# tomerlieber/doc-agents

Measured on AMD Instinct MI355X. Metric: QA queries/sec + p50 cache-miss latency; docs/min ingest at 1/2/4/8 MI355X, higher is better.
Workload: dtype bf16

## Files before the change

docagents_amd/ops/csrc/decode_attn.hip:

```cpp
#include "common.h"
#include "decode_merge.h"

#include <cstdlib>
#include <type_traits>

#pragma clang fp contract(on)

constexpr int DEC_NT = 1;
constexpr int DEC_VEARLY = 2;
constexpr int DEC_PFT = 4;
constexpr int DEC_XC = 8;

struct DecRope {
  bf16_t* kc;
  bf16_t* vc;
  const float* cs;
  const int* pos;
};

template <int D, int G, int VAR>
__global__ void __launch_bounds__(256)
decode_attn_kernel(const bf16_t* __restrict__ q, int ldq, const bf16_t* __restrict__ kc,
                   const bf16_t* __restrict__ vc, const int* __restrict__ lens, const int* __restrict__ slot,
                   const int* __restrict__ pre,
// ... 407 lines not shown
#pragma unroll
      for (int ds = 0; ds < NDS; ++ds) sacc[t] = mfma16(__builtin_bit_cast(bf16x8_t, kr[t][ds]), qf[ds], sacc[t]);
    }
    float mx = -INFINITY;
#pragma unroll
    for (int t = 0; t < 4; ++t)
#pragma unroll
      for (int i = 0; i < 4; ++i) {
        const int key = 16 * t + 4 * fg + i;
        const float sc = key < nk ? sacc[t][i] * scale_log2e : -INFINITY;
        sacc[t][i] = sc;
        mx = fmaxf(mx, sc);
      }
    mx = fmaxf(mx, __shfl_xor(mx, 16, 64));
    mx = max_xhalf(mx);
    const float m_new = fmaxf(m_run, mx);
    const float m_use = (m_new == -INFINITY) ? 0.f : m_new;
    const float alpha = exp2f(m_run - m_use);
    m_run = m_new;
    float psum = 0.f;
#pragma unroll
    for (int t = 0; t < 4; ++t)
#pragma unroll
      for (int i = 0; i < 4; ++i) {
        const float p = __builtin_amdgcn_exp2f(sacc[t][i] - m_use);
        sacc[t][i] = p;
        psum += p;
      }
    l_part = l_part * alpha + psum;
#pragma unroll
    for (int i = 0; i < NDT; ++i) oacc[i] *= alpha;
    asm volatile("s_waitcnt vmcnt(0)" ::: "memory");
#pragma unroll
    for (int c = 0; c < 2; ++c) {
      const u32x4_t pw = u32x4_t{pack_bf2(sacc[2 * c][0], sacc[2 * c][1]), pack_bf2(sacc[2 * c][2], sacc[2 * c][3]),
                                 pack_bf2(sacc[2 * c + 1][0], sacc[2 * c + 1][1]),
                                 pack_bf2(sacc[2 * c + 1][2], sacc[2 * c + 1][3])};
      const bf16x8_t pb = __builtin_bit_cast(bf16x8_t, pw);
      const int q4 = fr >> 2, p4 = fr & 3;
#pragma unroll
      for (int dt = 0; dt < NDT; ++dt) {
        const int col = dt * 16 + 4 * p4;
        const int r0 = 32 * c + 4 * fg + q4, r1 = r0 + 16;
        const s16x4_t lo = lds_read_tr16(myv + r0 * (D * 2) + (((col >> 3) ^ vswz<D>(r0)) << 4) + (col & 7) * 2);
        const s16x4_t hi = lds_read_tr16(myv + r1 * (D * 2) + (((col >> 3) ^ vswz<D>(r1)) << 4) + (col & 7) * 2);
        const bf16x8_t va = bf16x8_t{lo[0], lo[1], lo[2], lo[3], hi[0], hi[1], hi[2], hi[3]};
        oacc[dt] = mfma16(va, pb, oacc[dt]);
      }
    }
    asm volatile("s_waitcnt lgkmcnt(0)" ::: "memory");
  }
  float l_tot = l_part + __shfl_xor(l_part, 16, 64);
  l_tot = sum_xhalf(l_tot);
  if (fg == 0) { swm[w][fr] = m_run; swl[w][fr] = l_tot; }
  __syncthreads();
  float* so = (float*)sv;
#pragma unroll
  for (int dt = 0; dt < NDT; ++dt)
#pragma unroll
    for (int i = 0; i < 4; ++i) so[(w * 16 + fr) * D + dt * 16 + 4 * fg + i] = oacc[dt][i];
  __syncthreads();
  for (int i = tid; i < G * D; i += 256) {
    const int g = i / D, d = i % D;
    const float M = fmaxf(fmaxf(swm[0][g], swm[1][g]), fmaxf(swm[2][g], swm[3][g]));
    const float Mu = (M == -INFINITY) ? 0.f : M;
    float o = 0.f, ls = 0.f;
#pragma unroll
    for (int ww = 0; ww < 4; ++ww) {
      const float f = exp2f(swm[ww][g] - Mu);
      o += so[(ww * 16 + g) * D + d] * f;
      ls += swl[ww][g] * f;
    }
    dec_store(o, M, ls, b, hk * G + g, d, H, nsplit, split, D, po, pm, pl, out, ldo);
  }
  __shared__ int s_last;
  dec_finish<D, G>(po, pm, pl, H, Hkv, nsplit, b, hk, cnt, out, ldo, &s_last);
}

template <int D>
__device__ __forceinline__ int vswz1(int r) {
  return D == 96 ? ((r >> 1) & 3) : vswz<D>(r);
}

template <int D, bool XC, bool RP>
__global__ void __launch_bounds__(256)
decode_attn_mfma1_kernel(const bf16_t* __restrict__ q, int ldq, const bf16_t* __restrict__ kc,
                         const bf16_t* __restrict__ vc, const int* __restrict__ lens, const int* __restrict__ slot,
                         const int* __restrict__ pre, int H, int Hkv, int max_seq, int chunk_max, int nsplit,
                         float scale_log2e, float* __restrict__ po, float* __restrict__ pm, float* __restrict__ pl,
                         bf16_t* __restrict__ out, int ldo, int* __restrict__ cnt, DecRope rope) {
  static_assert(D == 64 || D == 96 || D == 128, "head dim");
  constexpr int KT = 64, NDS = D / 32, NDT = D / 16, NS = D / 8;
  constexpr int VBYTES = KT * D * 2, NDMA = VBYTES / 1024;
  typedef __attribute__((address_space(3))) void* lds_ptr_t;
  typedef __attribute__((address_space(1))) const void* gptr_t;
  __shared__ __attribute__((aligned(16))) char sv[4 * 2 * VBYTES];
  __shared__ float swm[4], swl[4];

  int split = blockIdx.x, hk = blockIdx.y, b = blockIdx.z;
  if constexpr (XC) {
    const int wl = blockIdx.x + gridDim.x * (blockIdx.y + gridDim.y * blockIdx.z);
    const int s8 = wl >> 3, pair = (s8 / nsplit) * 8 + (wl & 7);
    split = s8 % nsplit;
    hk = pair % Hkv;
    b = pair / Hkv;
  }
  const int L = lens[b];
  DA_ASSERT(L >= 0 && L <= max_seq && slot[b] >= 0);
  const int chunk = dec_chunk(L, nsplit, chunk_max);
  DA_ASSERT(chunk <= 8 * KT);
  const int kstart = split * chunk;
  const bool own_new = RP && kstart <= L - 1 && L - 1 < kstart + chunk;
  const int kend = min(RP ? L - 1 : L, kstart + chunk);
  const int tid = threadIdx.x, lane = tid & 63, w = tid >> 6;
  const int fr = lane & 15, fg = lane >> 4;
  const size_t cbase = ((size_t)slot[b] * Hkv + hk) * (size_t)max_seq * D;
  const int P = pre ? pre[2 * b] : 0;
  const size_t pbase = P ? ((size_t)pre[2 * b + 1] * Hkv + hk) * (size_t)max_seq * D : cbase;
  DA_ASSERT(P >= 0 && P <= L);
  DA_ASSERT(!RP || rope.pos[b] == L - 1);

  const int ta = kstart + w * KT, tb = ta + 4 * KT;
  u32x4_t kr[2][4][NDS];
  auto issue_tile = [&](auto STR, int j, int t0) {
    constexpr bool S = decltype(STR)::value;
    const int nk = kend - t0;
    const bool shared = t0 < P;
    const bf16_t* kb = nk > 0 ? kc + (shared ? pbase : cbase) + (size_t)t0 * D : kc + cbase;
    const bf16_t* vb = nk > 0 ? vc + (shared ? pbase : cbase) + (size_t)t0 * D : vc + cbase;
    const int last = nk > 0 ? min(KT, nk) - 1 : 0;
    [[maybe_unused]] const int npre = P - t0;
    [[maybe_unused]] const bf16_t* ko = kc + cbase + (size_t)t0 * D;
    [[maybe_unused]] const bf16_t* vo = vc + cbase + (size_t)t0 * D;
#pragma unroll
    for (int t = 0; t < 4; ++t)
#pragma unroll
      for (int ds = 0; ds < NDS; ++ds) {
        const int key = min(16 * t + fr, last);
        const bf16_t* base = (S && key >= npre) ? ko : kb;
        kr[j][t][ds] = __builtin_nontemporal_load((const u32x4_t*)(base + (size_t)key * D + ds * 32 + fg * 8));
      }
    char* myv = sv + (w * 2 + j) * VBYTES;
#pragma unroll
    for (int i = 0; i < NDMA; ++i) {
      const int pc = i * 64 + lane, row = pc / NS, sl = pc % NS;
      const int c = sl ^ vswz1<D>(row);
      const int key = min(row, last);
      const bf16_t* base = (S && key >= npre) ? vo : vb;
      __builtin_amdgcn_global_load_lds((gptr_t)(base + (size_t)key * D + c * 8), (lds_ptr_t)(myv + i * 1024), 16, 0, 2);
    }
  };
  auto issue = [&](int j, int t0) {
    if (t0 < P && P < t0 + KT && t0 < kend) issue_tile(std::true_type{}, j, t0);
    else issue_tile(std::false_type{}, j, t0);
  };
  issue(0, ta);
  issue(1, tb);

  bf16x8_t qf[NDS];
  [[maybe_unused]] __shared__ __attribute__((aligned(16))) bf16_t sqb[RP ? D : 1];
  [[maybe_unused]] __shared__ float skn[RP ? D : 1], svn[RP ? D : 1];
  [[maybe_unused]] __shared__ float ssn;
  if constexpr (RP) {
    constexpr int HALF = D / 2;
    const bf16_t* qrow = q + (size_t)b * ldq;
    if (tid < D) {
      const int d = tid, i = d >> 1;
      const float c = rope.cs[((size_t)(L - 1) * HALF + i) * 2], sn = rope.cs[((size_t)(L - 1) * HALF + i) * 2 + 1];
      auto rot = [&](const bf16_t* hp) {
        const float x1 = bf2f(hp[d & ~1]), x2 = bf2f(hp[d | 1]);
        return f2bf((d & 1) ? x2 * c + x1 * sn : x1 * c - x2 * sn);
      };
      sqb[d] = rot(qrow + hk * D);
      if (own_new) {
        const bf16_t kn = rot(qrow + (size_t)(H + hk) * D), vn = qrow[(size_t)(H + Hkv + hk) * D + d];
        skn[d] = bf2f(kn);
        svn[d] = bf2f(vn);
        const size_t crow = cbase + (size_t)(L - 1) * D;
        rope.kc[crow + d] = kn;
        rope.vc[crow + d] = vn;
      }
    }
    __syncthreads();
#pragma unroll
    for (int ds = 0; ds < NDS; ++ds)
      qf[ds] = fr == 0 ? *(const bf16x8_t*)(sqb + ds * 32 + fg * 8) : bf16x8_t{0, 0, 0, 0, 0, 0, 0, 0};
    if (own_new && w == 0) {
      float part = 0.f;
      for (int d = lane; d < D; d += 64) part += bf2f(sqb[d]) * skn[d];
      part = wave_sum(part);
      if (lane == 0) ssn = part * scale_log2e;
    }
  } else {
#pragma unroll
    for (int ds = 0; ds < NDS; ++ds)
      qf[ds] = fr == 0 ? *(const bf16x8_t*)(q + (size_t)b * ldq + hk * D + ds * 32 + fg * 8)
                       : bf16x8_t{0, 0, 0, 0, 0, 0, 0, 0};
  }
  f32x4_t oacc[NDT];
#pragma unroll
  for (int i = 0; i < NDT; ++i) oacc[i] = f32x4_t{0.f, 0.f, 0.f, 0.f};
  float m_run = -INFINITY, l_part = 0.f;
  asm volatile("s_waitcnt vmcnt(0)" ::: "memory");

  auto process = [&](int j, int t0) {
    const int nk = kend - t0;
    f32x4_t sacc[4];
#pragma unroll
    for (int t = 0; t < 4; ++t) {
      sacc[t] = f32x4_t{0.f, 0.f, 0.f, 0.f};
#pragma unroll
      for (int ds = 0; ds < NDS; ++ds) sacc[t] = mfma16(__builtin_bit_cast(bf16x8_t, kr[j][t][ds]), qf[ds], sacc[t]);
    }
    float mx = -INFINITY;
#pragma unroll
    for (int t = 0; t < 4; ++t)
#pragma unroll
      for (int i = 0; i < 4; ++i) {
        const int key = 16 * t + 4 * fg + i;
        const float sc = key < nk ? sacc[t][i] * scale_log2e : -INFINITY;
        sacc[t][i] = sc;
        mx = fmaxf(mx, sc);
      }
    mx = fmaxf(mx, __shfl_xor(mx, 16, 64));
    mx = max_xhalf(mx);
    const float m_new = fmaxf(m_run, mx);
    const float m_use = (m_new == -INFINITY) ? 0.f : m_new;
    const float alpha = exp2f(m_run - m_use);
    m_run = m_new;
    float psum = 0.f;
#pragma unroll
    for (int t = 0; t < 4; ++t)
#pragma unroll
      for (int i = 0; i < 4; ++i) {
        const float p = __builtin_amdgcn_exp2f(sacc[t][i] - m_use);
        sacc[t][i] = p;
        psum += p;
      }
    l_part = l_part * alpha + psum;
#pragma unroll
    for (int i = 0; i < NDT; ++i) oacc[i] *= alpha;
    const char* myv = sv + (w * 2 + j) * VBYTES;
#pragma unroll
    for (int c = 0; c < 2; ++c) {
      const u32x4_t pw = u32x4_t{pack_bf2(sacc[2 * c][0], sacc[2 * c][1]), pack_bf2(sacc[2 * c][2], sacc[2 * c][3]),
                                 pack_bf2(sacc[2 * c + 1][0], sacc[2 * c + 1][1]),
                                 pack_bf2(sacc[2 * c + 1][2], sacc[2 * c + 1][3])};
      const bf16x8_t pb = __builtin_bit_cast(bf16x8_t, pw);
      const int q4 = fr >> 2, p4 = fr & 3;
#pragma unroll
      for (int dt = 0; dt < NDT; ++dt) {
        const int col = dt * 16 + 4 * p4;
        const int r0 = 32 * c + 4 * fg + q4, r1 = r0 + 16;
        const s16x4_t lo = lds_read_tr16(myv + r0 * (D * 2) + (((col >> 3) ^ vswz1<D>(r0)) << 4) + (col & 7) * 2);
        const s16x4_t hi = lds_read_tr16(myv + r1 * (D * 2) + (((col >> 3) ^ vswz1<D>(r1)) << 4) + (col & 7) * 2);
        const bf16x8_t va = bf16x8_t{lo[0], lo[1], lo[2], lo[3], hi[0], hi[1], hi[2], hi[3]};
        oacc[dt] = mfma16(va, pb, oacc[dt]);
      }
    }
  };
  if (ta < kend) process(0, ta);
  if (tb < kend) process(1, tb);

  float l_tot = l_part + __shfl_xor(l_part, 16, 64);
  l_tot = sum_xhalf(l_tot);
  if (lane == 0) { swm[w] = m_run; swl[w] = l_tot; }
  asm volatile("s_waitcnt lgkmcnt(0)" ::: "memory");
  __syncthreads();
  float* so = (float*)sv;
  if (fr == 0) {
#pragma unroll
    for (int dt = 0; dt < NDT; ++dt)
#pragma unroll
      for (int i = 0; i < 4; ++i) so[w * D + dt * 16 + 4 * fg + i] = oacc[dt][i];
  }
  __syncthreads();
  for (int d = tid; d < D; d += 256) {
    float M = fmaxf(fmaxf(swm[0], swm[1]), fmaxf(swm[2], swm[3]));
    if (own_new) M = fmaxf(M, ssn);
    const float Mu = (M == -INFINITY) ? 0.f : M;
    float o = 0.f, ls = 0.f;
#pragma unroll
    for (int ww = 0; ww < 4; ++ww) {
      const float f = exp2f(swm[ww] - Mu);
      o += so[ww * D + d] * f;
      ls += swl[ww] * f;
    }
    if (own_new) {
      const float f = exp2f(ssn - Mu);
      o += svn[d] * f;
      ls += f;
    }
    dec_store(o, M, ls, b, hk, d, H, nsplit, split, D, po, pm, pl, out, ldo);
  }
  __shared__ int s_last;
  dec_finish<D, 1, XC>(po, pm, pl, H, Hkv, nsplit, b, hk, cnt, out, ldo, &s_last);
}

constexpr int kDecPrefetchPairs = 32;
enum DecRoute { DEC_INVALID, DEC_MFMA1, DEC_MHA_STREAM, DEC_MHA_PREFETCH, DEC_MHA_PREFETCH_XC, DEC_GQA_MFMA, DEC_GQA_VALU };

static DecRoute dec_route(int D, int G, int pairs, int chunk, int nsplit, bool has_rope, bool xc, bool has_cnt,
                          bool mfma1_enabled) {
  const bool few = pairs <= kDecPrefetchPairs;
  if (G == 1) {
    if (xc && (!few || pairs % 8 || !has_cnt || nsplit < 2)) return DEC_INVALID;
    if (mfma1_enabled && few && chunk <= 512) return DEC_MFMA1;
    if (xc) return DEC_MHA_PREFETCH_XC;
    return few ? DEC_MHA_PREFETCH : DEC_MHA_STREAM;
  }
  if (xc || has_rope || (G != 2 && G != 4 && G != 8)) return DEC_INVALID;
  return D == 96 ? DEC_GQA_VALU : DEC_GQA_MFMA;
}

struct DecBf16Args : DecArgs {
  const bf16_t* kc; const bf16_t* vc;
  DecRope rope;
};

template <int D>
static int launch_decode(const DecBf16Args& a, DecRoute route, bool xc) {
#define VALU(GG, VAR) decode_attn_kernel<D, GG, VAR><<<a.grid, 256, 0, a.s>>>(a.q, a.ldq, a.kc, a.vc, DEC_KARGS(a), a.rope)
#define GQA(GG) decode_attn_gqa_kernel<D, GG><<<a.grid, 256, 0, a.s>>>(a.q, a.ldq, a.kc, a.vc, DEC_KARGS(a))
#define M1(XCV, RPV) decode_attn_mfma1_kernel<D, XCV, RPV><<<a.grid, 256, 0, a.s>>>(a.q, a.ldq, a.kc, a.vc, DEC_KARGS(a), a.rope)
  const bool rp = a.rope.cs != nullptr;
  switch (route) {
    case DEC_MFMA1:
      if (xc) { if (rp) M1(true, true); else M1(true, false); }
      else { if (rp) M1(false, true); else M1(false, false); }
      break;
    case DEC_MHA_STREAM: VALU(1, DEC_NT | DEC_VEARLY); break;
    case DEC_MHA_PREFETCH: VALU(1, DEC_NT | DEC_VEARLY | DEC_PFT); break;
    case DEC_MHA_PREFETCH_XC: VALU(1, DEC_NT | DEC_VEARLY | DEC_PFT | DEC_XC); break;
    case DEC_GQA_MFMA:
      if constexpr (D != 96) { if (a.G == 2) GQA(2); else if (a.G == 4) GQA(4); else GQA(8); }
      else return (int)hipErrorInvalidValue;
      break;
    case DEC_GQA_VALU:
      if constexpr (D == 96) { if (a.G == 2) VALU(2, DEC_NT); else if (a.G == 4) VALU(4, DEC_NT); else VALU(8, DEC_NT); }
      else return (int)hipErrorInvalidValue;
      break;
    default: return (int)hipErrorInvalidValue;
  }
#undef VALU
#undef GQA
#undef M1
  return (int)hipGetLastError();
}

DA_EXPORT int da_malloc_uncached(long long bytes, void** out) {
  hipError_t e = hipExtMallocWithFlags(out, (size_t)bytes, hipDeviceMallocUncached);
  if (e != hipSuccess) return (int)e;
  e = hipMemset(*out, 0, (size_t)bytes);
  if (e != hipSuccess) return (int)e;
  return (int)hipDeviceSynchronize();
}

DA_EXPORT int da_decode_attn(const void* q, int ldq, const void* k_cache, const void* v_cache, const void* lens,
                             const void* slot, const void* pre, int B, int H, int Hkv, int D, int max_seq, int chunk,
                             int nsplit, float scale, void* ws, void* o, int ldo, void* counters, const void* cos_sin,
                             const void* pos, int xc, void* stream) {
  DecBf16Args a;
  if (dec_fill(a, q, ldq, lens, slot, pre, B, H, Hkv, D, max_seq, chunk, nsplit, scale, ws, o, ldo, counters, cos_sin,
               pos, stream) || !k_cache || !v_cache)
    return (int)hipErrorInvalidValue;
  if (B == 0) return 0;
  a.kc = (const bf16_t*)k_cache; a.vc = (const bf16_t*)v_cache;
  a.rope = DecRope{(bf16_t*)k_cache, (bf16_t*)v_cache, (const float*)cos_sin, (const int*)pos};
  static const char* const m1 = getenv("DA_DECODE_MFMA1");
  const DecRoute route = dec_route(D, a.G, B * Hkv, chunk, nsplit, cos_sin != nullptr, xc != 0, counters != nullptr,
                                   !(m1 && m1[0] == '0'));
  const int err = D == 64 ? launch_decode<64>(a, route, xc != 0)
                  : D == 96 ? launch_decode<96>(a, route, xc != 0) : launch_decode<128>(a, route, xc != 0);
  return err ? err : dec_combine(a);
}
```

docagents_amd/ops/csrc/decode_merge.h:

```cpp
#pragma once
#include "common.h"

__device__ __forceinline__ int dec_chunk(int L, int nsplit, int chunk_arg) {
  const int c = ((L + nsplit - 1) / nsplit + 63) & ~63;
  return c < chunk_arg ? c : chunk_arg;
}

__device__ __forceinline__ void dec_store(float o, float M, float ls, int b, int h, int d, int H, int nsplit,
                                          int split, int D, float* po, float* pm, float* pl, bf16_t* out,
                                          int ldo) {
  if (nsplit == 1) {
    out[(size_t)b * ldo + h * D + d] = f2bf(ls > 0.f ? o / ls : 0.f);
    return;
  }
  const size_t pidx = ((size_t)b * H + h) * nsplit + split;
  po[pidx * D + d] = o;
  if (d == 0) { pm[pidx] = M; pl[pidx] = ls; }
}

template <int D, int G, bool XC = false>
__device__ __forceinline__ void dec_finish(const float* po, const float* pm, const float* pl, int H, int Hkv,
                                           int nsplit, int b, int hk, int* cnt, bf16_t* out, int ldo, int* s_last) {
  if (nsplit == 1 || cnt == nullptr) return;
  const int tid = threadIdx.x;
  asm volatile("s_waitcnt vmcnt(0)" ::: "memory");
  __syncthreads();
  if (tid == 0) {
    int* c = &cnt[b * Hkv + hk];
    const int old = XC ? __hip_atomic_fetch_add(c, 1, __ATOMIC_RELAXED, __HIP_MEMORY_SCOPE_AGENT) : atomicAdd(c, 1);
    *s_last = old == nsplit - 1;
    if (*s_last) {
      if constexpr (XC) __hip_atomic_store(c, 0, __ATOMIC_RELAXED, __HIP_MEMORY_SCOPE_AGENT);
      else *c = 0;
    }
  }
  __syncthreads();
  if (!*s_last) return;
  auto ld = [](const float* p) -> float {
    if constexpr (XC) return __hip_atomic_load(p, __ATOMIC_RELAXED, __HIP_MEMORY_SCOPE_AGENT);
    else return *p;
  };
  for (int i = tid; i < G * D; i += blockDim.x) {
    const int g = i / D, d = i % D, h = hk * G + g;
    const size_t base = ((size_t)b * H + h) * nsplit;
    float M = -INFINITY, lsum = 0.f, acc = 0.f;
    for (int s0 = 0; s0 < nsplit; s0 += 8) {
      float ms[8], ls[8], os[8];
#pragma unroll
      for (int j = 0; j < 8; ++j) {
        const int s = min(s0 + j, nsplit - 1);
        ms[j] = ld(pm + base + s);
        ls[j] = ld(pl + base + s);
        os[j] = ld(po + (base + s) * D + d);
      }
      float mx = M;
#pragma unroll
      for (int j = 0; j < 8; ++j)
        if (s0 + j < nsplit) mx = fmaxf(mx, ms[j]);
      const float mu = (mx == -INFINITY) ? 0.f : mx;
      const float r = (M == -INFINITY) ? 0.f : exp2f(M - mu);
      lsum *= r;
      acc *= r;
#pragma unroll
      for (int j = 0; j < 8; ++j) {
        if (s0 + j >= nsplit) continue;
        const float f = exp2f(ms[j] - mu);
        lsum += ls[j] * f;
        acc += os[j] * f;
      }
      M = mx;
    }
    out[(size_t)b * ldo + h * D + d] = f2bf(lsum > 0.f ? acc / lsum : 0.f);
  }
}

template <int D>
__global__ void decode_combine_kernel(const float* __restrict__ po, const float* __restrict__ pm,
                                      const float* __restrict__ pl, int H, int nsplit, bf16_t* __restrict__ o,
                                      int ldo) {
  const int b = blockIdx.y, h = blockIdx.x;
  const size_t base = ((size_t)b * H + h) * nsplit;
  float M = -INFINITY;
  for (int s = 0; s < nsplit; ++s) M = fmaxf(M, pm[base + s]);
  const float Mu = (M == -INFINITY) ? 0.f : M;
  float lsum = 0.f;
  for (int s = 0; s < nsplit; ++s) lsum += pl[base + s] * exp2f(pm[base + s] - Mu);
  const float inv = lsum > 0.f ? 1.f / lsum : 0.f;
  for (int d = threadIdx.x; d < D; d += blockDim.x) {
    float acc = 0.f;
    for (int s = 0; s < nsplit; ++s) acc += po[(base + s) * D + d] * exp2f(pm[base + s] - Mu);
    o[(size_t)b * ldo + h * D + d] = f2bf(acc * inv);
  }
}

struct DecArgs {
  const bf16_t* q; const int* lens; const int* slot; const int* pre;
  int ldq, B, H, Hkv, G, D, max_seq, chunk, nsplit, ldo;
  float sl2e;
  float* po; float* pm; float* pl;
  bf16_t* out; int* cnt;
  dim3 grid;
  hipStream_t s;
};
#define DEC_KARGS(a) (a).lens, (a).slot, (a).pre, (a).H, (a).Hkv, (a).max_seq, (a).chunk, (a).nsplit, (a).sl2e, (a).po, \
                     (a).pm, (a).pl, (a).out, (a).ldo, (a).cnt

static inline int dec_fill(DecArgs& a, const void* q, int ldq, const void* lens, const void* slot, const void* pre,
                           int B, int H, int Hkv, int D, int max_seq, int chunk, int nsplit, float scale, void* ws,
                           void* o, int ldo, void* counters, const void* cos_sin, const void* pos, void* stream) {
  bool ok = Hkv >= 1 && H % Hkv == 0 && chunk >= 64 && chunk % 64 == 0 && nsplit >= 1 && (D == 64 || D == 96 || D == 128);
  ok = ok && q && lens && slot && o && (nsplit == 1 || ws);
  ok = ok && (cos_sin == nullptr) == (pos == nullptr) && (!cos_sin || (H == Hkv && ldq >= (H + 2 * Hkv) * D));
  if (!ok) return (int)hipErrorInvalidValue;
  a.q = (const bf16_t*)q; a.lens = (const int*)lens; a.slot = (const int*)slot; a.pre = (const int*)pre;
  a.ldq = ldq; a.B = B; a.H = H; a.Hkv = Hkv; a.G = H / Hkv; a.D = D; a.max_seq = max_seq; a.chunk = chunk;
  a.nsplit = nsplit; a.ldo = ldo;
  a.sl2e = scale * 1.4426950408889634f;
  a.po = (float*)ws; a.pm = a.po + (size_t)B * H * nsplit * D; a.pl = a.pm + (size_t)B * H * nsplit;
  a.out = (bf16_t*)o; a.cnt = (int*)counters;
  a.grid = dim3(nsplit, Hkv, B); a.s = (hipStream_t)stream;
  return 0;
}

static inline int dec_combine(const DecArgs& a) {
  if (a.nsplit == 1 || a.cnt) return 0;
#define DEC_COMBINE(DD, NT) decode_combine_kernel<DD><<<dim3(a.H, a.B), NT, 0, a.s>>>(a.po, a.pm, a.pl, a.H, a.nsplit, a.out, a.ldo)
  if (a.D == 64) DEC_COMBINE(64, 64); else if (a.D == 96) DEC_COMBINE(96, 128); else DEC_COMBINE(128, 128);
#undef DEC_COMBINE
  DA_LAUNCH_CHECK();
}
```

docagents_amd/ops/kernels.py:

```python
from __future__ import annotations

import contextlib
import ctypes
import math
import os
import threading
from pathlib import Path

import torch

from . import gemm_plan
from .gemm_plan import (DK_MAX_M, DK_SPLITK_ABOVE, dk_fusable, dk_parts, dk_w8_fusable,
                        gemv_fusable, gemv_w4_fusable, gemv_w8_fusable, keeps_w4_copy, keeps_w8_copy,
                        prefill_w8_fusable, tile_w8_fusable, weight_op)
from .reference import (dequant_mxfp4, quant_weight_fp8, quant_weight_fp8_pow2,
                        quant_weight_mxfp4)

_LIB = None
_LOCK = threading.Lock()
_DEBUG = os.environ.get("DA_KERNELS_DEBUG", "0") == "1"
_LIB_PATH = Path(__file__).resolve().parent / ("_da_kernels_debug.so" if _DEBUG else "_da_kernels.so")

EPI_NONE, EPI_BIAS, EPI_GELU, EPI_SWIGLU, EPI_RESID = 0, 1, 2, 3, 4
EPI_ROPE = 6
# ... 773 lines not shown
    max_seq = 0
    if k_cache is not None:
        _i32(slot, "slot")
        _req(k_cache.is_contiguous() and v_cache.is_contiguous() and k_cache.shape == v_cache.shape, "caches")
        _req(k_cache.dim() == 4 and k_cache.shape[1] == Hkv and k_cache.shape[3] == D, "cache [S, Hkv, max_seq, D]")
        max_seq = k_cache.shape[2]
    _check(lib().da_rope_cache(_ptr(qkv), _ptr(pos), _ptr(slot), _ptr(cos_sin), _ptr(k_cache), _ptr(v_cache),
                               T, H, Hkv, D, max_seq, 1 if rotate_q else 0, _stream()), "rope_cache")
    return qkv


def flash_kv_cache_ok(D: int, causal: bool) -> bool:
    return causal and D == 96


def flash_attn_varlen(q, k, v, cu_seqlens, max_seqlen: int, H: int, Hkv: int, D: int, causal: bool,
                      scale: float | None = None, out=None, prefix=None, kv_cache=None, tail_only: bool = False):
    kc = vc = ks = kpos = None
    if kv_cache is not None:
        kc, vc, ks, kpos = kv_cache
        _req(flash_kv_cache_ok(D, causal), "kv_cache: causal D = 96 only")
        _bf16_cuda(kc, "k_cache"); _bf16_cuda(vc, "v_cache"); _i32(ks, "slot"); _i32(kpos, "pos")
        _req(kc.is_contiguous() and vc.is_contiguous() and kc.shape == vc.shape and kc.dim() == 4
             and kc.shape[1] == Hkv and kc.shape[3] == D, "caches [slots, Hkv, max_seq, D]")
        _req(ks.numel() >= q.shape[0] and kpos.numel() >= q.shape[0], "slot / pos per token")
        k = v = q
    for t, n in ((q, "q"), (k, "k"), (v, "v")):
        _bf16_cuda(t, n)
        _req(t.dim() == 2 and t.stride(1) == 1 and t.stride(0) % 8 == 0 and t.data_ptr() % 16 == 0, f"{n} layout")
    _i32(cu_seqlens, "cu_seqlens")
    _req(D in (32, 64, 96, 128), f"head dim {D} unsupported")
    _req(H % Hkv == 0, "H % Hkv")
    T = q.shape[0]
    if out is None:
        out = torch.empty((T, H * D), dtype=torch.bfloat16, device=q.device)
    scale = scale if scale is not None else 1.0 / math.sqrt(D)
    B = cu_seqlens.numel() - 1
    kp = vp = None
    hstride, P = 0, 0
    if prefix is not None:
        kp, vp, P = prefix
        P = int(P)
        _bf16_cuda(kp, "k_pre"); _bf16_cuda(vp, "v_pre")
        _req(kp.dim() == 3 and kp.shape == vp.shape and kp.shape[0] == Hkv and kp.shape[2] == D
             and kp.is_contiguous() and vp.is_contiguous() and 0 <= P <= kp.shape[1], "prefix K/V [Hkv, max_seq, D]")
        hstride = kp.shape[1] * D
    if kc is not None:
        _req(prefix is None or kp.shape[1] == kc.shape[2], "prefix and caches differ in max_seq")
        hstride = kc.shape[2] * D
    _check(lib().da_flash_attn_v2(_ptr(q), _ptr(k), _ptr(v), q.stride(0), k.stride(0), v.stride(0),
                                  _ptr(cu_seqlens), B, int(max_seqlen), H, Hkv, D, int(causal), float(scale),
                                  _ptr(out), out.stride(0), _ptr(kp), _ptr(vp), hstride, P, _ptr(ks), _ptr(kpos),
                                  _ptr(kc), _ptr(vc), int(bool(tail_only)), _stream()),
           "flash_attn_varlen")
    return out


_FUSED_COMBINE = True
_UC: dict = {}


class _RawBuf:

    def __init__(self, ptr: int, nbytes: int):
        self.ptr, self.nbytes = ptr, nbytes

    def data_ptr(self) -> int:
        return self.ptr


def _uncached(tag: str, nbytes: int, device) -> _RawBuf:
    key = (tag, device.index if device.index is not None else torch.cuda.current_device(),
           getattr(_ROLE, "name", "main"))
    bufs = _UC.setdefault(key, [])
    if not bufs or bufs[-1].nbytes < nbytes:
        n = max(nbytes, 1 << 20)
        p = ctypes.c_void_p()
        with torch.cuda.device(device):
            _check(lib().da_malloc_uncached(n, ctypes.byref(p)), "hipExtMallocWithFlags(uncached)")
        bufs.append(_RawBuf(p.value, n))
    return bufs[-1]


def _decode_split(B: int, Hkv: int, max_len: int, chunk: int):
    if chunk <= 0:
        want = max_len * B * Hkv / 768
        chunk = 512
        while chunk < want and chunk < 4096:
            chunk *= 2
    return chunk, max(1, math.ceil(max_len / chunk))


DECODE_XC = os.environ.get("DA_DECODE_XC", "1") != "0"
MASKED_STREAMS = False
_XC_PROBE: dict = {}


def decode_xc_ok(device) -> bool:
    if not DECODE_XC or MASKED_STREAMS:
        return False
    idx = device.index if device.index is not None else torch.cuda.current_device()
    if idx in _XC_PROBE:
        return _XC_PROBE[idx]
    if torch.cuda.is_current_stream_capturing():
        return False
    n = 1024
    out = torch.zeros(n * 4, dtype=torch.int32, device=device)
    _check(lib().da_placement_probe(_ptr(out), n, 0, _stream()), "placement_probe")
    xcc = out.view(n, 4)[:, 0].cpu().numpy()
    ok = bool(len(set(xcc.tolist())) == 8 and all(len(set(xcc[r::8].tolist())) == 1 for r in range(8)))
    _XC_PROBE[idx] = ok
    return ok


_COUNTERS: dict = {}


def _cached_counters(tag: str, n: int, device) -> torch.Tensor:
    key = (tag, device.index if device.index is not None else torch.cuda.current_device(),
           getattr(_ROLE, "name", "main"))
    bufs = _COUNTERS.setdefault(key, [])
    if not bufs or bufs[-1].numel() < n:
        bufs.append(torch.zeros(max(n, 1024), dtype=torch.int32, device=device))
    return bufs[-1]


def _decode_operands(q, lens, slot, H, Hkv, D, max_len, max_seq, chunk, out, pre, rope=None):
    _bf16_cuda(q, "q"); _i32(lens, "lens"); _i32(slot, "slot")
    _req(D in (64, 96, 128), "head dim")
    _req(H % Hkv == 0 and (H // Hkv) in (1, 2, 4, 8), "GQA group must be 1/2/4/8")
    _req(q.dim() == 2 and q.stride(1) == 1 and q.shape[1] >= H * D, "q [B, >= H*D]")
    B = q.shape[0]
    _req(lens.numel() >= B and slot.numel() >= B, "lens / slot length")
    _req(0 < max_len <= max_seq, "max_len > cache capacity")
    if pre is not None:
        _i32(pre, "pre"); _req(pre.shape == (B, 2) and pre.is_contiguous(), "pre must be int32 [B, 2]")
    cs = ps = None
    if rope is not None:
        cs, ps = rope
        _req(H == Hkv and D % 8 == 0, "fused RoPE decode: MHA only")
        _i32(ps, "pos")
        _req(cs.dtype == torch.float32 and cs.is_contiguous() and cs.shape[1] == D // 2 and cs.shape[2] == 2, "cos_sin")
        _req(q.shape[1] >= (H + 2 * Hkv) * D, "fused RoPE decode needs the qkv row")
    chunk, nsplit = _decode_split(B, Hkv, max_len, chunk)
    _req(chunk % 64 == 0, "chunk must be a multiple of 64")
    if out is None:
        out = torch.empty((B, H * D), dtype=torch.bfloat16, device=q.device)
    _bf16_cuda(out, "out")
    _req(out.dim() == 2 and out.shape[0] == B and out.shape[1] >= H * D and out.stride(1) == 1, "out [B, >= H*D]")
    return chunk, nsplit, out, cs, ps


def _decode_buffers(B, H, Hkv, D, nsplit, device, same_xcd_ok: bool):
    nws = B * H * nsplit * (D + 2) * 4
    ws = _workspace(nws, device)
    if not (_FUSED_COMBINE and nsplit > 1):
        return ws, None, 0
    if same_xcd_ok and H == Hkv and B * Hkv <= 32 and (B * Hkv) % 8 == 0 and decode_xc_ok(device):
        return ws, _cached_counters("decode_cnt_xc", B * Hkv, device), 1
    cnt = _uncached("decode_cnt", B * Hkv * 4, device)
    return _uncached("decode_ws", nws, device), cnt, 0


def decode_attn(q, k_cache, v_cache, lens, slot, H, Hkv, D, max_len: int, chunk: int = 0, scale=None, out=None,
                pre=None, rope=None):
    _req(k_cache.dim() == 4 and k_cache.shape[1] == Hkv and k_cache.shape[3] == D, "cache shape")
    _req(rope is None or (k_cache.is_contiguous() and v_cache.is_contiguous()), "caches must be contiguous")
    chunk, nsplit, out, cs, ps = _decode_operands(q, lens, slot, H, Hkv, D, max_len, k_cache.shape[2], chunk, out, pre,
                                                  rope)
    B = q.shape[0]
    scale = scale if scale is not None else 1.0 / math.sqrt(D)
    ws, cnt, xc = _decode_buffers(B, H, Hkv, D, nsplit, q.device, same_xcd_ok=True)
    _check(lib().da_decode_attn(_ptr(q), q.stride(0), _ptr(k_cache), _ptr(v_cache), _ptr(lens), _ptr(slot), _ptr(pre), B, H,
                                Hkv, D, k_cache.shape[2], chunk, nsplit, float(scale), _ptr(ws), _ptr(out), out.stride(0),
                                _ptr(cnt), _ptr(cs), _ptr(ps), xc, _stream()), "decode_attn")
    return out


def _kv8_cache_checks(k_codes, v_codes, k_scale, v_scale, Hkv, D):
    for c, s, n in ((k_codes, k_scale, "k"), (v_codes, v_scale, "v")):
        _req(c.is_cuda and c.dtype in (FP8, torch.uint8) and c.is_contiguous(), f"{n}_codes must be contiguous e4m3 on GPU")
        _req(c.dim() == 4 and c.shape[1] == Hkv and c.shape[3] == D, f"{n}_codes [slots, Hkv, max_seq, D]")
        _req(s.is_cuda and s.dtype == torch.float32 and s.is_contiguous() and s.shape == c.shape[:3],
             f"{n}_scale must be contiguous fp32 [slots, Hkv, max_seq]")
        _req(c.data_ptr() % 16 == 0 and s.data_ptr() % 4 == 0, f"{n} cache alignment")
    _req(k_codes.shape == v_codes.shape, "k / v caches differ in shape")


def rope_cache_kv8(qkv, pos, cos_sin, H, Hkv, D, slot, k_codes, v_codes, k_scale, v_scale, rotate_q=True):
    _bf16_cuda(qkv, "qkv"); _i32(pos, "pos"); _i32(slot, "slot")
    T = qkv.shape[0]
    _req(D in (64, 96, 128), "head dim")
    _req(qkv.is_contiguous() and qkv.shape[1] == (H + 2 * Hkv) * D and qkv.data_ptr() % 16 == 0, "qkv shape")
    _req(pos.numel() >= T and slot.numel() >= T, "pos / slot length")
    _req(cos_sin.is_cuda and cos_sin.dtype == torch.float32 and cos_sin.is_contiguous() and cos_sin.dim() == 3
         and cos_sin.shape[-1] == 2 and cos_sin.shape[1] == D // 2, "cos_sin must be fp32 [max_pos, D/2, 2]")
    _kv8_cache_checks(k_codes, v_codes, k_scale, v_scale, Hkv, D)
    _check(lib().da_rope_cache_kv8(_ptr(qkv), _ptr(pos), _ptr(slot), _ptr(cos_sin), _ptr(k_codes), _ptr(v_codes),
                                   _ptr(k_scale), _ptr(v_scale), T, H, Hkv, D, k_codes.shape[2],
                                   1 if rotate_q else 0, _stream()), "rope_cache_kv8")
    return qkv


def decode_attn_kv8(q, k_codes, v_codes, k_scale, v_scale, lens, slot, H, Hkv, D, max_len: int, chunk: int = 0,
                    scale=None, out=None, pre=None):
    _kv8_cache_checks(k_codes, v_codes, k_scale, v_scale, Hkv, D)
    chunk, nsplit, out, _, _ = _decode_operands(q, lens, slot, H, Hkv, D, max_len, k_codes.shape[2], chunk, out, pre)
    B = q.shape[0]
    scale = scale if scale is not None else 1.0 / math.sqrt(D)
    ws, cnt, _ = _decode_buffers(B, H, Hkv, D, nsplit, q.device, same_xcd_ok=False)
    _check(lib().da_decode_attn_kv8(_ptr(q), q.stride(0), _ptr(k_codes), _ptr(v_codes), _ptr(k_scale), _ptr(v_scale),
                                    _ptr(lens), _ptr(slot), _ptr(pre), B, H, Hkv, D, k_codes.shape[2], chunk, nsplit,
                                    float(scale), _ptr(ws), _ptr(out), out.stride(0), _ptr(cnt), _stream()),
           "decode_attn_kv8")
    return out


def kv8_dequant(codes, scale, slot: int, P: int):
    slot, P = int(slot), int(P)
    _req(codes.is_cuda and codes.dtype in (FP8, torch.uint8) and codes.is_contiguous() and codes.dim() == 4
         and codes.shape[3] % 16 == 0 and codes.data_ptr() % 16 == 0, "codes [slots, Hkv, max_seq, D]")
    _req(scale.is_cuda and scale.dtype == torch.float32 and scale.is_contiguous() and scale.shape == codes.shape[:3],
         "scale fp32 [slots, Hkv, max_seq]")
    S, Hkv, max_seq, D = codes.shape
    _req(0 <= slot < S and 0 <= P <= max_seq, "slot / P out of range")
    out = torch.empty((Hkv, P, D), dtype=torch.bfloat16, device=codes.device)
    _check(lib().da_kv8_dequant(_ptr(codes), _ptr(scale), slot, S, Hkv, P, D, max_seq, _ptr(out), _stream()),
           "kv8_dequant")
    return out


SAMPLE_CHUNKED_MAX_B = 64
_SAMPLE_WS: dict = {}


def _sample_ws(nfloats: int, device) -> torch.Tensor:
    key = (device.index if device.index is not None else torch.cuda.current_device(), getattr(_ROLE, "name", "main"))
    bufs = _SAMPLE_WS.setdefault(key, [])
    if not bufs or bufs[-1].numel() < nfloats:
        bufs.append(torch.empty(max(nfloats, 16384), dtype=torch.float32, device=device))
    return bufs[-1]


def sample(logits, temperature: float, seed: int, step: int = 0, out_tok=None, out_lp=None, conf=None,
           active=None, ctr=None, pos=None, lens=None, hist=None, start=None, eos=()):
    _bf16_cuda(logits, "logits")
    B, V = logits.shape
    _req(logits.stride(1) == 1 and logits.stride(0) % 8 == 0, "logits layout")
    dev = logits.device
    if out_tok is None:
        out_tok = torch.empty(B, dtype=torch.int32, device=dev)
    if out_lp is None:
        out_lp = torch.empty(B, dtype=torch.float32, device=dev)
    if conf is not None:
        _req(conf.dtype == torch.float32 and conf.shape == (B, 2), "conf must be fp32 [B, 2]")
    for t, n in ((active, "active"), (ctr, "ctr"), (pos, "pos"), (lens, "lens"), (start, "start")):
        if t is not None:
            _i32(t, n); _req(t.numel() >= B, f"{n} too short")
    hist_ld = 0
    if hist is not None:
        _i32(hist, "hist"); _req(hist.dim() == 2 and hist.shape[0] >= B, "hist [B, n]")
        _req(pos is not None and start is not None, "hist needs pos and start")
        hist_ld = hist.shape[1]
    e = list(eos)[:4] + [-1] * (4 - min(4, len(eos)))
    if B <= SAMPLE_CHUNKED_MAX_B and V >= 4096:
        ws = _sample_ws(B * ((V + 1023) // 1024) * 8, dev)
        _check(lib().da_sample_chunked(_ptr(logits), B, V, logits.stride(0), float(temperature), seed & 0xffffffff,
                                       step & 0xffffffff, _ptr(ctr), _ptr(ws), _ptr(out_tok), _ptr(out_lp),
                                       _ptr(conf), _ptr(active), _ptr(pos), _ptr(lens), _ptr(hist), _ptr(start),
                                       hist_ld, e[0], e[1], e[2], e[3], _stream()), "sample_chunked")
        return out_tok, out_lp
    _check(lib().da_sample(_ptr(logits), B, V, logits.stride(0), float(temperature), seed & 0xffffffff,
                           step & 0xffffffff, _ptr(ctr), _ptr(out_tok), _ptr(out_lp), _ptr(conf), _ptr(active),
                           _ptr(pos), _ptr(lens), _ptr(hist), _ptr(start), hist_ld, e[0], e[1], e[2], e[3],
                           _stream()), "sample")
    return out_tok, out_lp


def sample_partial(logits, temperature: float, seed: int, v0: int, step: int = 0, ctr=None, out=None):
    _bf16_cuda(logits, "logits")
    B, V = logits.shape
    _req(logits.stride(1) == 1, "logits rows must be contiguous")
    if ctr is not None:
        _i32(ctr, "ctr"); _req(ctr.numel() >= B, "ctr too short")
    if out is None:
        out = torch.empty((B, 8), dtype=torch.float32, device=logits.device)
    _req(out.dtype == torch.float32 and out.shape == (B, 8) and out.is_contiguous(), "stats must be fp32 [B, 8]")
    _check(lib().da_sample_partial(_ptr(logits), B, V, logits.stride(0), int(v0), float(temperature),
                                   seed & 0xffffffff, step & 0xffffffff, _ptr(ctr), _ptr(out), _stream()),
           "sample_partial")
# ... 354 lines not shown
```

Before: 35.50.

## Add single-tile MFMA decode variant with smaller chunks for few-pair MHA decode

Adds a TILES template parameter to the MFMA1 MHA decode kernel so each wave can process one 64-key tile instead of two, halving LDS use and K registers. The host splitter now picks a 256-key chunk when batch×kv-heads is small (bf16 MHA only), which raises the split count and the number of workgroups. It routes those chunks to the single-tile variant. The fused split-combine is widened to 16 splits per batch, with all loads issued ahead of the math behind a scheduling barrier. The aim is more parallelism and occupancy for small-batch decode, at the cost of more partial results to merge.

```diff
diff --git a/docagents_amd/ops/csrc/decode_attn.hip b/docagents_amd/ops/csrc/decode_attn.hip
--- a/docagents_amd/ops/csrc/decode_attn.hip
+++ b/docagents_amd/ops/csrc/decode_attn.hip
@@ -513,7 +513,7 @@
   return D == 96 ? ((r >> 1) & 3) : vswz<D>(r);
 }
 
-template <int D, bool XC, bool RP>
+template <int D, bool XC, bool RP, int TILES>
 __global__ void __launch_bounds__(256)
 decode_attn_mfma1_kernel(const bf16_t* __restrict__ q, int ldq, const bf16_t* __restrict__ kc,
                          const bf16_t* __restrict__ vc, const int* __restrict__ lens, const int* __restrict__ slot,
@@ -521,11 +521,12 @@
                          float scale_log2e, float* __restrict__ po, float* __restrict__ pm, float* __restrict__ pl,
                          bf16_t* __restrict__ out, int ldo, int* __restrict__ cnt, DecRope rope) {
   static_assert(D == 64 || D == 96 || D == 128, "head dim");
+  static_assert(TILES == 1 || TILES == 2, "tiles per wave");
   constexpr int KT = 64, NDS = D / 32, NDT = D / 16, NS = D / 8;
   constexpr int VBYTES = KT * D * 2, NDMA = VBYTES / 1024;
   typedef __attribute__((address_space(3))) void* lds_ptr_t;
   typedef __attribute__((address_space(1))) const void* gptr_t;
-  __shared__ __attribute__((aligned(16))) char sv[4 * 2 * VBYTES];
+  __shared__ __attribute__((aligned(16))) char sv[4 * TILES * VBYTES];
   __shared__ float swm[4], swl[4];
 
   int split = blockIdx.x, hk = blockIdx.y, b = blockIdx.z;
@@ -539,11 +540,12 @@
   const int L = lens[b];
   DA_ASSERT(L >= 0 && L <= max_seq && slot[b] >= 0);
   const int chunk = dec_chunk(L, nsplit, chunk_max);
-  DA_ASSERT(chunk <= 8 * KT);
+  DA_ASSERT(chunk <= 4 * TILES * KT);
   const int kstart = split * chunk;
   const bool own_new = RP && kstart <= L - 1 && L - 1 < kstart + chunk;
   const int kend = min(RP ? L - 1 : L, kstart + chunk);
-  const int tid = threadIdx.x, lane = tid & 63, w = tid >> 6;
+  const int tid = threadIdx.x, lane = tid & 63;
+  const int w = __builtin_amdgcn_readfirstlane(tid >> 6);
   const int fr = lane & 15, fg = lane >> 4;
   const size_t cbase = ((size_t)slot[b] * Hkv + hk) * (size_t)max_seq * D;
   const int P = pre ? pre[2 * b] : 0;
@@ -552,14 +554,14 @@
   DA_ASSERT(!RP || rope.pos[b] == L - 1);
 
   const int ta = kstart + w * KT, tb = ta + 4 * KT;
-  u32x4_t kr[2][4][NDS];
+  u32x4_t kr[TILES][4][NDS];
   auto issue_tile = [&](auto STR, int j, int t0) {
     constexpr bool S = decltype(STR)::value;
     const int nk = kend - t0;
     const bool shared = t0 < P;
-    const bf16_t* kb = nk > 0 ? kc + (shared ? pbase : cbase) + (size_t)t0 * D : kc + cbase;
-    const bf16_t* vb = nk > 0 ? vc + (shared ? pbase : cbase) + (size_t)t0 * D : vc + cbase;
-    const int last = nk > 0 ? min(KT, nk) - 1 : 0;
+    const bf16_t* kb = kc + (shared ? pbase : cbase) + (size_t)t0 * D;
+    const bf16_t* vb = vc + (shared ? pbase : cbase) + (size_t)t0 * D;
+    const int last = min(KT, nk) - 1;
     [[maybe_unused]] const int npre = P - t0;
     [[maybe_unused]] const bf16_t* ko = kc + cbase + (size_t)t0 * D;
     [[maybe_unused]] const bf16_t* vo = vc + cbase + (size_t)t0 * D;
@@ -571,7 +573,7 @@
         const bf16_t* base = (S && key >= npre) ? ko : kb;
         kr[j][t][ds] = __builtin_nontemporal_load((const u32x4_t*)(base + (size_t)key * D + ds * 32 + fg * 8));
       }
-    char* myv = sv + (w * 2 + j) * VBYTES;
+    char* myv = sv + (w * TILES + j) * VBYTES;
 #pragma unroll
     for (int i = 0; i < NDMA; ++i) {
       const int pc = i * 64 + lane, row = pc / NS, sl = pc % NS;
@@ -582,11 +584,12 @@
     }
   };
   auto issue = [&](int j, int t0) {
-    if (t0 < P && P < t0 + KT && t0 < kend) issue_tile(std::true_type{}, j, t0);
+    if (t0 >= kend) return;
+    if (t0 < P && P < t0 + KT) issue_tile(std::true_type{}, j, t0);
     else issue_tile(std::false_type{}, j, t0);
   };
   issue(0, ta);
-  issue(1, tb);
+  if constexpr (TILES == 2) issue(1, tb);
 
   bf16x8_t qf[NDS];
   [[maybe_unused]] __shared__ __attribute__((aligned(16))) bf16_t sqb[RP ? D : 1];
@@ -671,7 +674,7 @@
     l_part = l_part * alpha + psum;
 #pragma unroll
     for (int i = 0; i < NDT; ++i) oacc[i] *= alpha;
-    const char* myv = sv + (w * 2 + j) * VBYTES;
+    const char* myv = sv + (w * TILES + j) * VBYTES;
 #pragma unroll
     for (int c = 0; c < 2; ++c) {
       const u32x4_t pw = u32x4_t{pack_bf2(sacc[2 * c][0], sacc[2 * c][1]), pack_bf2(sacc[2 * c][2], sacc[2 * c][3]),
@@ -691,7 +694,9 @@
     }
   };
   if (ta < kend) process(0, ta);
-  if (tb < kend) process(1, tb);
+  if constexpr (TILES == 2) {
+    if (tb < kend) process(1, tb);
+  }
 
   float l_tot = l_part + __shfl_xor(l_part, 16, 64);
   l_tot = sum_xhalf(l_tot);
@@ -725,18 +730,18 @@
     dec_store(o, M, ls, b, hk, d, H, nsplit, split, D, po, pm, pl, out, ldo);
   }
   __shared__ int s_last;
-  dec_finish<D, 1, XC>(po, pm, pl, H, Hkv, nsplit, b, hk, cnt, out, ldo, &s_last);
+  dec_finish<D, 1, XC, TILES == 1 ? 16 : 8>(po, pm, pl, H, Hkv, nsplit, b, hk, cnt, out, ldo, &s_last);
 }
 
 constexpr int kDecPrefetchPairs = 32;
-enum DecRoute { DEC_INVALID, DEC_MFMA1, DEC_MHA_STREAM, DEC_MHA_PREFETCH, DEC_MHA_PREFETCH_XC, DEC_GQA_MFMA, DEC_GQA_VALU };
+enum DecRoute { DEC_INVALID, DEC_MFMA1, DEC_MFMA1_T1, DEC_MHA_STREAM, DEC_MHA_PREFETCH, DEC_MHA_PREFETCH_XC, DEC_GQA_MFMA, DEC_GQA_VALU };
 
 static DecRoute dec_route(int D, int G, int pairs, int chunk, int nsplit, bool has_rope, bool xc, bool has_cnt,
                           bool mfma1_enabled) {
   const bool few = pairs <= kDecPrefetchPairs;
   if (G == 1) {
     if (xc && (!few || pairs % 8 || !has_cnt || nsplit < 2)) return DEC_INVALID;
-    if (mfma1_enabled && few && chunk <= 512) return DEC_MFMA1;
+    if (mfma1_enabled && few && chunk <= 512) return chunk <= 256 ? DEC_MFMA1_T1 : DEC_MFMA1;
     if (xc) return DEC_MHA_PREFETCH_XC;
     return few ? DEC_MHA_PREFETCH : DEC_MHA_STREAM;
   }
@@ -753,12 +758,16 @@
 static int launch_decode(const DecBf16Args& a, DecRoute route, bool xc) {
 #define VALU(GG, VAR) decode_attn_kernel<D, GG, VAR><<<a.grid, 256, 0, a.s>>>(a.q, a.ldq, a.kc, a.vc, DEC_KARGS(a), a.rope)
 #define GQA(GG) decode_attn_gqa_kernel<D, GG><<<a.grid, 256, 0, a.s>>>(a.q, a.ldq, a.kc, a.vc, DEC_KARGS(a))
-#define M1(XCV, RPV) decode_attn_mfma1_kernel<D, XCV, RPV><<<a.grid, 256, 0, a.s>>>(a.q, a.ldq, a.kc, a.vc, DEC_KARGS(a), a.rope)
+#define M1(XCV, RPV, T) decode_attn_mfma1_kernel<D, XCV, RPV, T><<<a.grid, 256, 0, a.s>>>(a.q, a.ldq, a.kc, a.vc, DEC_KARGS(a), a.rope)
   const bool rp = a.rope.cs != nullptr;
   switch (route) {
     case DEC_MFMA1:
-      if (xc) { if (rp) M1(true, true); else M1(true, false); }
-      else { if (rp) M1(false, true); else M1(false, false); }
+      if (xc) { if (rp) M1(true, true, 2); else M1(true, false, 2); }
+      else { if (rp) M1(false, true, 2); else M1(false, false, 2); }
+      break;
+    case DEC_MFMA1_T1:
+      if (xc) { if (rp) M1(true, true, 1); else M1(true, false, 1); }
+      else { if (rp) M1(false, true, 1); else M1(false, false, 1); }
       break;
     case DEC_MHA_STREAM: VALU(1, DEC_NT | DEC_VEARLY); break;
     case DEC_MHA_PREFETCH: VALU(1, DEC_NT | DEC_VEARLY | DEC_PFT); break;
diff --git a/docagents_amd/ops/csrc/decode_merge.h b/docagents_amd/ops/csrc/decode_merge.h
--- a/docagents_amd/ops/csrc/decode_merge.h
+++ b/docagents_amd/ops/csrc/decode_merge.h
@@ -18,7 +18,7 @@
   if (d == 0) { pm[pidx] = M; pl[pidx] = ls; }
 }
 
-template <int D, int G, bool XC = false>
+template <int D, int G, bool XC = false, int SB = 8>
 __device__ __forceinline__ void dec_finish(const float* po, const float* pm, const float* pl, int H, int Hkv,
                                            int nsplit, int b, int hk, int* cnt, bf16_t* out, int ldo, int* s_last) {
   if (nsplit == 1 || cnt == nullptr) return;
@@ -44,25 +44,27 @@
     const int g = i / D, d = i % D, h = hk * G + g;
     const size_t base = ((size_t)b * H + h) * nsplit;
     float M = -INFINITY, lsum = 0.f, acc = 0.f;
-    for (int s0 = 0; s0 < nsplit; s0 += 8) {
-      float ms[8], ls[8], os[8];
+    for (int s0 = 0; s0 < nsplit; s0 += SB) {
+      float ms[SB], ls[SB], os[SB];
 #pragma unroll
-      for (int j = 0; j < 8; ++j) {
+      for (int j = 0; j < SB; ++j) {
         const int s = min(s0 + j, nsplit - 1);
         ms[j] = ld(pm + base + s);
         ls[j] = ld(pl + base + s);
-        os[j] = ld(po + (base + s) * D + d);
       }
+#pragma unroll
+      for (int j = 0; j < SB; ++j) os[j] = ld(po + (base + min(s0 + j, nsplit - 1)) * D + d);
+      __builtin_amdgcn_sched_barrier(0);
       float mx = M;
 #pragma unroll
-      for (int j = 0; j < 8; ++j)
+      for (int j = 0; j < SB; ++j)
         if (s0 + j < nsplit) mx = fmaxf(mx, ms[j]);
       const float mu = (mx == -INFINITY) ? 0.f : mx;
       const float r = (M == -INFINITY) ? 0.f : exp2f(M - mu);
       lsum *= r;
       acc *= r;
 #pragma unroll
-      for (int j = 0; j < 8; ++j) {
+      for (int j = 0; j < SB; ++j) {
         if (s0 + j >= nsplit) continue;
         const float f = exp2f(ms[j] - mu);
         lsum += ls[j] * f;
diff --git a/docagents_amd/ops/kernels.py b/docagents_amd/ops/kernels.py
--- a/docagents_amd/ops/kernels.py
+++ b/docagents_amd/ops/kernels.py
@@ -879,7 +879,14 @@
     return bufs[-1]
 
 
-def _decode_split(B: int, Hkv: int, max_len: int, chunk: int):
+DECODE_FEW_RULE = True
+DECODE_FEW_CHUNK = 256
+DECODE_FEW_PAIRS = 32
+
+
+def _decode_split(B: int, Hkv: int, max_len: int, chunk: int, few_ok: bool = True):
+    if chunk <= 0 and few_ok and DECODE_FEW_RULE and B * Hkv <= DECODE_FEW_PAIRS:
+        chunk = DECODE_FEW_CHUNK
     if chunk <= 0:
         want = max_len * B * Hkv / 768
         chunk = 512
@@ -922,7 +929,7 @@
     return bufs[-1]
 
 
-def _decode_operands(q, lens, slot, H, Hkv, D, max_len, max_seq, chunk, out, pre, rope=None):
+def _decode_operands(q, lens, slot, H, Hkv, D, max_len, max_seq, chunk, out, pre, rope=None, bf16_cache=True):
     _bf16_cuda(q, "q"); _i32(lens, "lens"); _i32(slot, "slot")
     _req(D in (64, 96, 128), "head dim")
     _req(H % Hkv == 0 and (H // Hkv) in (1, 2, 4, 8), "GQA group must be 1/2/4/8")
@@ -939,7 +946,7 @@
         _i32(ps, "pos")
         _req(cs.dtype == torch.float32 and cs.is_contiguous() and cs.shape[1] == D // 2 and cs.shape[2] == 2, "cos_sin")
         _req(q.shape[1] >= (H + 2 * Hkv) * D, "fused RoPE decode needs the qkv row")
-    chunk, nsplit = _decode_split(B, Hkv, max_len, chunk)
+    chunk, nsplit = _decode_split(B, Hkv, max_len, chunk, few_ok=bf16_cache and H == Hkv)
     _req(chunk % 64 == 0, "chunk must be a multiple of 64")
     if out is None:
         out = torch.empty((B, H * D), dtype=torch.bfloat16, device=q.device)
@@ -1002,7 +1009,8 @@
 def decode_attn_kv8(q, k_codes, v_codes, k_scale, v_scale, lens, slot, H, Hkv, D, max_len: int, chunk: int = 0,
                     scale=None, out=None, pre=None):
     _kv8_cache_checks(k_codes, v_codes, k_scale, v_scale, Hkv, D)
-    chunk, nsplit, out, _, _ = _decode_operands(q, lens, slot, H, Hkv, D, max_len, k_codes.shape[2], chunk, out, pre)
+    chunk, nsplit, out, _, _ = _decode_operands(q, lens, slot, H, Hkv, D, max_len, k_codes.shape[2], chunk, out, pre,
+                                                bf16_cache=False)
     B = q.shape[0]
     scale = scale if scale is not None else 1.0 / math.sqrt(D)
     ws, cnt, _ = _decode_buffers(B, H, Hkv, D, nsplit, q.device, same_xcd_ok=False)
```

After: 35.53, median of 2. About the same (+0.1%).
